# borglab/gtsfm

Hardware: NVIDIA H100
Metric: image_pairs_per_sec (higher is better)
Workload: dtype f32

## Files before the change

gtsfm_b200/_lib.py:

```python
from __future__ import annotations

import ctypes as C
from pathlib import Path
from typing import Optional

import numpy as np

LIB_PATH = Path(__file__).resolve().parent / "libgtsfm_b200.so"

_lib: Optional[C.CDLL] = None


class B200Error(RuntimeError):
    pass


class LightGlueParams(C.Structure):
    _fields_ = [("depth_confidence", C.c_double), ("width_confidence", C.c_double), ("filter_threshold", C.c_double),
                ("prune_min_kpts", C.c_int), ("fp16_attention", C.c_int)]


class LightGluePair(C.Structure):
    _fields_ = [("kp0", C.c_void_p), ("desc0", C.c_void_p), ("n0", C.c_int), ("kp1", C.c_void_p), ("desc1", C.c_void_p), ("n1", C.c_int),
                ("out_matches", C.c_void_p), ("out_scores", C.c_void_p), ("out_k", C.c_int), ("out_stop_layer", C.c_int),
# ... 128 lines not shown
class TwoViewEvalResult(C.Structure):
    _fields_ = [("num_rows", C.c_int), ("num_inliers_gt", C.c_int), ("no_gt", C.c_int), ("no_rows", C.c_int),
                ("inlier_avg_reproj_error_gt", C.c_double), ("outlier_avg_reproj_error_gt", C.c_double),
                ("R_error_deg", C.c_double), ("U_error_deg", C.c_double)]


class ViewGraphParams(C.Structure):
    _fields_ = [("criterion", C.c_int), ("pad_", C.c_int), ("error_threshold_deg", C.c_double)]


VG_MEDIAN, VG_MIN = 0, 1

_vp, _i, _f, _sz = C.c_void_p, C.c_int, C.c_float, C.c_size_t
_ip = C.POINTER(C.c_int)

SIGNATURES = {
    "b2_version": (_i, []),
    "b2_create": (_i, [_i, C.POINTER(_vp)]),
    "b2_destroy": (None, [_vp]),
    "b2_last_error": (C.c_char_p, [_vp]),
    "b2_launch_count": (C.c_uint64, [_vp]),
    "b2_h2d_bytes": (C.c_uint64, [_vp]),
    "b2_set_option": (C.c_int, [_vp, C.c_char_p, C.c_int64]),
    "b2_profile_start": (_i, [_vp, C.c_char_p]),
    "b2_profile_stop": (_i, [_vp, C.POINTER(C.c_double), C.POINTER(C.c_uint64), C.POINTER(C.c_double)]),
    "b2_debug_fetch": (C.c_int64, [_vp, C.c_char_p, _vp, C.c_int64]),
    "b2_debug_linear_host": (_i, [_vp, C.POINTER(LinearLaunch), C.POINTER(LinearProblem), _i]),
    "b2_debug_conv_host": (_i, [_vp, C.POINTER(ConvLayer)]),
    "b2_debug_gemm_segments_host": (_i, [_vp, _vp, _vp, _vp, _i, _i, _i, _i, _vp, _vp, _i, _vp, _vp]),
    "b2_debug_attention_host": (_i, [_vp, _i, _ip, _ip, _i, _f, _i, _vp, _vp, _vp, _vp]),
    "b2_debug_superglue_assign_host": (_i, [_vp, _i, _i, _vp, _i, _i, _f, _i, _f, _vp, _vp, _vp, _vp, _vp, _vp, _vp, _ip, _ip]),
    "b2_debug_lightglue_assign_host": (_i, [_vp, _i, _i, _vp, _i, _i, _vp, _vp, _vp, _vp, _f, _vp, _vp, _vp, _vp, _vp, _vp, _vp, _ip,
                                            _ip]),
    "b2_debug_lightglue_argmax_host": (_i, [_vp, _i, _vp, _i, _i, _vp, _vp, _vp, _vp, _vp, _ip]),
    "b2_debug_lightglue_posenc_host": (_i, [_vp, _i, _vp, _vp, _vp, _vp, _vp, _vp]),
    "b2_debug_lightglue_ln_gelu_host": (_i, [_vp, _i, _vp, _vp, _vp, _vp, _vp, _vp]),
    "b2_debug_lightglue_rowheads_host": (_i, [_vp, _i, _vp, _vp, _vp, _vp, _vp, _vp, _vp, _vp, _vp, _vp]),
    "b2_debug_lightglue_prune_host": (_i, [_vp, _i, _vp, _vp, _vp, _f, _f, _vp, _vp]),
    "b2_debug_lightglue_gather_host": (_i, [_vp, _i, _vp, _vp, _vp, _vp, _vp, _vp, _vp, _vp, _vp, _vp, _vp, _vp, _vp]),
    "b2_debug_lightglue_filter_host": (_i, [_vp, _i, _i, _vp, _vp, _vp, _f, _vp, _vp, _vp, _vp, _ip]),
    "b2_superpoint_set_weights": (_i, [_vp, _vp, _sz]),
    "b2_superpoint_detect_dev": (_i, [_vp, _vp, _i, _i, _i, _sz, _f, _i, _i, _vp, _vp, _i, _ip, C.POINTER(C.c_uint64), _vp]),
    "b2_superpoint_describe_dev": (_i, [_vp, C.c_uint64, _vp, _i, _vp, _vp]),
    "b2_superpoint_extract_dev": (_i, [_vp, _vp, _i, _i, _i, _sz, _f, _i, _i, _i, _vp, _vp, _vp, _ip, _vp]),
    "b2_superpoint_extract_async_dev": (_i, [_vp, _vp, _i, _i, _i, _sz, _f, _i, _i, _i, _vp, _vp, _vp, _vp, _vp]),
    "b2_superpoint_finish_dev": (_i, [_vp, _vp]),
    "b2_superpoint_detect_host": (_i, [_vp, _vp, _i, _i, _i, _f, _i, _i, _vp, _vp, _i, _ip, C.POINTER(C.c_uint64)]),
    "b2_superpoint_describe_host": (_i, [_vp, C.c_uint64, _vp, _i, _vp]),
    "b2_image_resize_dev": (_i, [_vp, _vp, _i, _i, _i, _sz, _vp, _i, _i, _vp]),
    "b2_lightglue_set_weights": (_i, [_vp, _vp, _sz]),
    "b2_lightglue_qkv_rows": (_i, [_vp]),
    "b2_lightglue_match_dev": (_i, [_vp, _vp, _vp, _i, _vp, _vp, _i, C.POINTER(LightGlueParams), _vp, _vp, _ip, _ip, _vp]),
    "b2_lightglue_match_host": (_i, [_vp, _vp, _vp, _i, _vp, _vp, _i, C.POINTER(LightGlueParams), _vp, _vp, _ip, _ip]),
    "b2_lightglue_match_batched_dev": (_i, [_vp, C.POINTER(LightGluePair), _i, C.POINTER(LightGlueParams), _vp]),
    "b2_lightglue_trace_count": (_i, [_vp]),
    "b2_lightglue_trace_get": (_i, [_vp, _i, _vp, _vp, _vp, _vp, _vp, _vp]),
    "b2_lightglue_encoded_bytes": (_sz, [_i]),
    "b2_lightglue_encode_batched_dev": (_i, [_vp, C.POINTER(LightGlueImage), _i, C.POINTER(LightGlueParams), _vp]),
    "b2_superglue_set_weights": (_i, [_vp, _vp, _sz]),
    "b2_superglue_match_dev": (_i, [_vp, _vp, _vp, _vp, _i, _i, _i, _vp, _vp, _vp, _i, _i, _i, _i, _f, _vp, _vp, _ip, _vp]),
    "b2_superglue_match_host": (_i, [_vp, _vp, _vp, _vp, _i, _i, _i, _vp, _vp, _vp, _i, _i, _i, _i, _f, _vp, _vp, _ip]),
    "b2_superglue_trace_count": (_i, [_vp]),
    "b2_superglue_trace_get": (_i, [_vp, _i, _vp, _vp]),
    "b2_netvlad_blob_floats": (_sz, []),
    "b2_netvlad_set_weights": (_i, [_vp, _vp, _sz]),
    "b2_netvlad_describe_dev": (_i, [_vp, _vp, _i, _i, _i, _vp, _vp]),
# ... 136 lines not shown
```

gtsfm_b200/csrc/lightglue.cu:

```cuda
#include <stdlib.h>

#include "common.cuh"
#include "linear.cuh"
#include "assign_ps.cuh"

namespace {
constexpr int LG_LAYERS = 9;
constexpr size_t LG_NFLOATS = 11851601;
constexpr int D = 256;

struct SelfW {
  float *wqkv, *bqkv, *wout, *bout, *w0, *b0, *lng, *lnb, *w3, *b3;
};
struct CrossW {
  float *wqv, *bqv, *wout, *bout, *w0, *b0, *lng, *lnb, *w3, *b3;
};
struct AssignW {
  float *wm, *bm, *wf, *bf;
};
struct ConfW {
  float *w, *b;
};
}

// ... 7 lines not shown
  int n = 0;
  int cap = 0;
};

struct LgPair {
  bool active = false;
  int n0 = 0, n1 = 0;
  int stop = 0;
  long long* out_matches = nullptr;
  float* out_scores = nullptr;
};

struct LgTraceRec {
  int pair = 0, side = 0, layer = 0, n = 0;
  int heads = 0;
  int unconf = 0, kept = 0, stop = 0;
  std::vector<float> x, conf, mat;
  std::vector<int> ind, keep;
};

struct LightGlueState {
  bool loaded = false;
  int persist_ctas = 132;
  DevBuf wblob, wblob_h, wblob_l, errflag;
  bool use_tc = true;
  float* wr = nullptr;
  SelfW sw[LG_LAYERS];
  CrossW cw[LG_LAYERS];
  AssignW aw[LG_LAYERS];
  ConfW tw[LG_LAYERS - 1];
  float thr[LG_LAYERS];
  LgSide side[LG_MAX_SIDES];
  LgPair pair[LG_MAX_PAIRS];
  DevBuf sim[LG_MAX_PAIRS], counters, attn_part, attn_ml, attn_cnt, as_part, as_bar;
  HostBuf hread;
  std::vector<LgTraceRec> trace;
};

template <typename J>
struct JobList {
  J j[LG_MAX_SIDES];
};

void lg_destroy(b2_context* ctx) {
  delete ctx->lg;
  ctx->lg = nullptr;
}


struct PosJob {
  const float* kp;
  int n;
  float *cs, *sn;
  int* ind;
};
__global__ void __launch_bounds__(1024) k_lg_posenc(const __grid_constant__ JobList<PosJob> jobs, const float* __restrict__ wr ) {
  const PosJob& jb = jobs.j[blockIdx.y];
  const float* __restrict__ kp = jb.kp;
  const int n = jb.n;
  float* __restrict__ cs = jb.cs;
  float* __restrict__ sn = jb.sn;
  int* __restrict__ ind = jb.ind;
  if (n <= 0 || blockIdx.x * 1024 >= n * 32) return;
  __shared__ float red[4][32];
  __shared__ float bb[4];
  float mnx = INFINITY, mny = INFINITY, mxx = -INFINITY, mxy = -INFINITY;
  for (int i = threadIdx.x; i < n; i += blockDim.x) {
// ... 365 lines not shown
  if (j < n) {
    const float cm = cmax[j], cl = clog[j], l1 = l1g[j];
    for (int i0 = warp; i0 < m; i0 += LG_COL_WARPS * LG_COL_UNROLL) {
      float x[LG_COL_UNROLL], rm[LG_COL_UNROLL], rl[LG_COL_UNROLL], l0[LG_COL_UNROLL];
#pragma unroll
      for (int u = 0; u < LG_COL_UNROLL; ++u) {
        const int i = i0 + u * LG_COL_WARPS;
        const bool in = i < m;
        x[u] = in ? sim[(size_t)i * n + j] : 0.f;
        rm[u] = in ? rmax[i] : 0.f, rl[u] = in ? rlog[i] : 0.f, l0[u] = in ? l0g[i] : 0.f;
      }
#pragma unroll
      for (int u = 0; u < LG_COL_UNROLL; ++u) {
        const int i = i0 + u * LG_COL_WARPS;
        if (i < m) {
          const float sc = (((x[u] - rm[u]) - rl[u]) + ((x[u] - cm) - cl)) + (l0[u] + l1);
          if (sc > bv) bv = sc, bi = i;
        }
      }
    }
  }
  sv[warp][lane] = bv, si[warp][lane] = bi;
  __syncthreads();
  if (warp == 0 && j < n) {
    for (int w = 1; w < LG_COL_WARPS; ++w) {
      float ov = sv[w][lane];
      int oi = si[w][lane];
      if (ov > bv || (ov == bv && oi < bi)) bv = ov, bi = oi;
    }
    arg[j] = bi == 0x7fffffff ? 0 : bi;
  }
}

__global__ void __launch_bounds__(1024) k_lg_filter(const float* __restrict__ best0, const int* __restrict__ a0,
                                                     const int* __restrict__ a1, int m, float th, const int* __restrict__ ind0,
                                                     const int* __restrict__ ind1, long long* __restrict__ out,
                                                     float* __restrict__ outs, int* __restrict__ count) {
  __shared__ int wtot[32];
  __shared__ int carry;
  if (threadIdx.x == 0) carry = 0;
  __syncthreads();
  const int lane = threadIdx.x & 31, warp = threadIdx.x >> 5;
  for (int base = 0; base < m; base += 1024) {
    int i = base + threadIdx.x;
    bool valid = false;
    float ms = 0.f;
    int j = 0;
    if (i < m) {
      j = a0[i];
      bool mutual = a1[j] == i;
      ms = mutual ? expf(best0[i]) : 0.f;
      valid = mutual && best0[i] > -INFINITY && ms > th;
    }
    unsigned vm = __ballot_sync(0xffffffffu, valid);
    if (lane == 0) wtot[warp] = __popc(vm);
    __syncthreads();
    if (warp == 0) {
      int w = wtot[lane], ws = w;
#pragma unroll
      for (int o = 1; o < 32; o <<= 1) {
        int u = __shfl_up_sync(0xffffffffu, ws, o);
        if (lane >= o) ws += u;
      }
      wtot[lane] = ws - w;
    }
    __syncthreads();
    int pos = carry + wtot[warp] + __popc(vm & ((1u << lane) - 1));
    if (valid) {
      out[2 * (size_t)pos] = ind0[i];
      out[2 * (size_t)pos + 1] = ind1[j];
      if (outs) outs[pos] = ms;
    }
    __syncthreads();
    if (threadIdx.x == 1023) carry = pos + (valid ? 1 : 0);
    __syncthreads();
  }
  if (threadIdx.x == 0) *count = carry;
}


struct LgStats {
  float *max, *log, *lsg;
};
struct LgAssign {
  const float* sim;
  int M, N;
  const float *z0, *z1;
  const int *ind0, *ind1;
  float thr;
  LgStats r, c;
  float* best0;
  int *arg0, *arg1;
  DevBuf *part, *bar;
  int* err_flag;
  long long* out_matches;
  float* out_scores;
  int* count;
};

static int lg_assign_argmax(b2_context* ctx, cudaStream_t st, const LgAssign& p, int path, int G, int* ran) {
  const float* sim = p.sim;
  const int M = p.M, N = p.N;
  const bool persistent = path == 0 ? assign_ps_fits(1, N) : path == 1;
  if (persistent && !assign_ps_fits(1, N)) return b2_fail(ctx, B2_ERR_ARG, "the persistent assignment kernel holds at most 6240 columns");
  if (ran) *ran = persistent ? 1 : 2;
  int rc;
  if (persistent) {
    B2_CUDA(ctx, p.part->ensure((size_t)G * 2 * N * sizeof(float)));
    B2_CUDA(ctx, p.bar->ensure(16));
    B2_CUDA(ctx, cudaMemsetAsync(p.bar->p, 0, 16, st));
    SinkArgs sa{};
    sa.Z = sim, sa.M = M, sa.N = N, sa.iters = 1, sa.u = p.r.max, sa.v = p.c.max;
    sa.rlog = p.r.log, sa.clog = p.c.log, sa.z0 = p.z0, sa.z1 = p.z1;
    sa.lsg0 = p.r.lsg, sa.lsg1 = p.c.lsg, sa.part = p.part->as<float>(), sa.bar = p.bar->as<unsigned>();
    sa.best0 = p.best0, sa.arg0 = p.arg0, sa.arg1 = p.arg1, sa.err_flag = p.err_flag;
    if ((rc = launch_assign_ps<1>(ctx, st, sa, G, "k_lg_assign"))) return rc;
  } else {
    B2_LAUNCH(ctx, k_lg_row_stats, cdiv(M, 8), 256, 0, st, sim, M, N, p.r.max, p.r.log, p.z0, p.r.lsg);
    B2_CHECK_LAUNCH(ctx);
    B2_LAUNCH(ctx, k_lg_col_stats, cdiv(N, 32), 1024, 0, st, sim, M, N, p.c.max, p.c.log, p.z1, p.c.lsg);
    B2_CHECK_LAUNCH(ctx);
    B2_LAUNCH(ctx, k_lg_row_argmax, cdiv(M, 8), 256, 0, st, sim, M, N, p.r.max, p.r.log, p.c.max, p.c.log, p.r.lsg, p.c.lsg, p.best0,
              p.arg0);
    B2_CHECK_LAUNCH(ctx);
    B2_LAUNCH(ctx, k_lg_col_argmax, cdiv(N, 32), 1024, 0, st, sim, M, N, p.r.max, p.r.log, p.c.max, p.c.log, p.r.lsg, p.c.lsg, p.arg1);
    B2_CHECK_LAUNCH(ctx);
  }
  return B2_OK;
}

static int lg_assign(b2_context* ctx, cudaStream_t st, const LgAssign& p, int path, int G, int* ran) {
  const int M = p.M;
  int rc;
  if ((rc = lg_assign_argmax(ctx, st, p, path, G, ran))) return rc;
  B2_LAUNCH(ctx, k_lg_filter, 1, 1024, 0, st, p.best0, p.arg0, p.arg1, M, p.thr, p.ind0, p.ind1, p.out_matches, p.out_scores, p.count);
  B2_CHECK_LAUNCH(ctx);
  return B2_OK;
}

extern "C" int b2_lightglue_qkv_rows(int* out) {
  if (!out) return B2_ERR_ARG;
  for (int r = 0; r < 3 * D; ++r) out[r] = (r % D) * 3 + r / D;
  return B2_OK;
}

extern "C" int b2_lightglue_set_weights(b2_context* ctx, const float* blob, size_t n_floats) {
  if (!ctx || !blob) return B2_ERR_ARG;
  std::lock_guard<std::mutex> lk(ctx->mu);
  if (n_floats != LG_NFLOATS)
    return b2_fail(ctx, B2_ERR_ARG, "lightglue blob must hold 11851601 floats, got " + std::to_string(n_floats));
  cudaSetDevice(ctx->device);
  if (!ctx->lg) ctx->lg = new LightGlueState();
  LightGlueState* s = ctx->lg;
  std::vector<size_t> sizes;
  sizes.push_back(64);
  for (int i = 0; i < LG_LAYERS; ++i) {
    const size_t self_sz[] = {768 * 256, 768, 256 * 256, 256, 512 * 512, 512, 512, 512, 256 * 512, 256};
    const size_t cross_sz[] = {256 * 256, 256, 256 * 256, 256, 256 * 256, 256, 512 * 512, 512, 512, 512, 256 * 512, 256};
    for (size_t z : self_sz) sizes.push_back(z);
    for (size_t z : cross_sz) sizes.push_back(z);
  }
  for (int i = 0; i < LG_LAYERS; ++i) {
    const size_t asz[] = {256, 1, 256 * 256, 256};
    for (size_t z : asz) sizes.push_back(z);
  }
  for (int i = 0; i < LG_LAYERS - 1; ++i) sizes.push_back(256), sizes.push_back(1);
  constexpr int SELF_T = 10, LAYER_T = 22;
  std::vector<size_t> order(sizes.size());
// ... 399 lines not shown
    int ns = 0, mx = 0;
    for (int li = 0; li < nlive; ++li) {
      if (s->pair[live[li]].stop != layer) continue;
      for (int side = 0; side < 2; ++side) {
        LgSide& sd = s->side[2 * live[li] + side];
        const float* x = sd.x[sd.cur].as<float>();
        LinArgs& a = g[ns];
        a.a1f = x, a.a1p = planes_of(sd.xs[sd.cur], (size_t)sd.cap * 256), a.lda1 = 256, a.K1 = 256, a.w = s->aw[layer].wf, a.ldb = 256;
        a.bias = s->aw[layer].bf, a.scale = 0.25f;
        a.cf = sd.md.as<float>(), a.ldc = 256, a.cp = planes_of(sd.md, (size_t)sd.cap * 256), a.ldch = 256, a.M = sd.n, a.N = 256;
        hj.j[ns] = {x, sd.n, s->aw[layer].wm, s->aw[layer].bm, nullptr, nullptr, sd.ls.as<float>()};
        mx = sd.n > mx ? sd.n : mx;
        ++ns;
      }
    }
    if (ns == 0) continue;
    if ((rc = run_linear(ctx, st, tw, g, ns, "lg_assign_proj"))) return rc;
    B2_LAUNCH(ctx, k_lg_rowheads, dim3(cdiv(mx, 8), ns), 256, 0, st, hj, (const float*)nullptr, (const float*)nullptr);
    B2_CHECK_LAUNCH(ctx);
  }
  {
    LinArgs gs[LG_MAX_PAIRS];
    for (int li = 0; li < nlive; ++li) {
      const int p = live[li];
      LgSide &a = s->side[2 * p], &b = s->side[2 * p + 1];
      B2_CUDA(ctx, s->sim[p].ensure((size_t)a.n * b.n * 4));
      LinArgs& g = gs[li];
      g.a1f = a.md.as<float>(), g.a1p = planes_of(a.md, (size_t)a.cap * 256), g.lda1 = 256, g.K1 = 256;
      g.bf = b.md.as<float>(), g.bp = planes_of(b.md, (size_t)b.cap * 256), g.ldb = 256;
      g.cf = s->sim[p].as<float>(), g.ldc = b.n, g.tc_want_f32 = true, g.M = a.n, g.N = b.n;
    }
    if ((rc = run_linear(ctx, st, tw, gs, nlive, "lg_assign_sim"))) return rc;
  }
  for (int li = 0; li < nlive; ++li) {
    const int p = live[li];
    LgSide &a = s->side[2 * p], &b = s->side[2 * p + 1];
    const LgAssign la{s->sim[p].as<float>(), a.n, b.n, a.ls.as<float>(), b.ls.as<float>(), a.ind[a.cur].as<int>(), b.ind[b.cur].as<int>(),
                      (float)prm->filter_threshold, {a.rmax.as<float>(), a.rlog.as<float>(), a.lsg.as<float>()},
                      {b.rmax.as<float>(), b.rlog.as<float>(), b.lsg.as<float>()}, a.amax.as<float>(), a.aidx.as<int>(), b.aidx.as<int>(),
                      &s->as_part, &s->as_bar, s->errflag.as<int>(), s->pair[p].out_matches, s->pair[p].out_scores,
                      counters + 4 * LG_MAX_PAIRS + p};
    if ((rc = lg_assign(ctx, st, la, 0, s->persist_ctas, nullptr))) return rc;
  }
  B2_CUDA(ctx, cudaMemcpyAsync(hread + 4 * LG_MAX_PAIRS, counters + 4 * LG_MAX_PAIRS, LG_MAX_PAIRS * sizeof(int), cudaMemcpyDeviceToHost, st));
  B2_CUDA(ctx, cudaMemcpyAsync(hread + 5 * LG_MAX_PAIRS, s->errflag.p, sizeof(int), cudaMemcpyDeviceToHost, st));
  B2_CUDA(ctx, cudaStreamSynchronize(st));
  if (s->use_tc && hread[5 * LG_MAX_PAIRS]) return b2_fail(ctx, B2_ERR_STATE, "wgmma pipeline timed out on an mbarrier (kernel bug)");
  for (int li = 0; li < nlive; ++li) pairs[live[li]].out_k = hread[4 * LG_MAX_PAIRS + live[li]];
  ctx->debug["lg_desc0"] = {s->side[0].x[s->side[0].cur].as<float>(), (int64_t)s->side[0].n * 256};
  ctx->debug["lg_desc1"] = {s->side[1].x[s->side[1].cur].as<float>(), (int64_t)s->side[1].n * 256};
  return B2_OK;
}

static int lg_match_pairs(b2_context* ctx, b2_lightglue_pair* pairs, int n_pairs, const b2_lightglue_params* prm, cudaStream_t st) {
  LightGlueState* s = ctx->lg;
  if (!s || !s->loaded) return b2_fail(ctx, B2_ERR_STATE, "lightglue weights not set");
  s->persist_ctas = ctx->sm_count - ctx->reserve_sms > 0 ? ctx->sm_count - ctx->reserve_sms : 1;
  s->trace.clear();
  const int bmax = ctx->lg_batch > 0 && ctx->lg_batch < LG_MAX_PAIRS ? ctx->lg_batch : LG_MAX_PAIRS;
  for (int p0 = 0; p0 < n_pairs; p0 += bmax) {
    const int np = n_pairs - p0 < bmax ? n_pairs - p0 : bmax;
    int rc = lg_match_batch(ctx, pairs + p0, np, prm, st, p0);
    if (rc) return rc;
  }
  return B2_OK;
}

extern "C" int b2_lightglue_match_batched_dev(b2_context* ctx, b2_lightglue_pair* pairs, int n_pairs, const b2_lightglue_params* params,
                                              void* stream) {
  if (!ctx || !params || n_pairs < 0 || (n_pairs > 0 && !pairs)) return B2_ERR_ARG;
  for (int p = 0; p < n_pairs; ++p) {
    const b2_lightglue_pair& pr = pairs[p];
    if (pr.n0 < 0 || pr.n1 < 0) return B2_ERR_ARG;
    if (pr.n0 > 0 && pr.n1 > 0 && (!pr.kp0 || !pr.desc0 || !pr.kp1 || !pr.desc1 || !pr.out_matches)) return B2_ERR_ARG;
    if (((uintptr_t)pr.enc0 | (uintptr_t)pr.enc1) & 15) return B2_ERR_ARG;
  }
// ... 175 lines not shown
  std::vector<int> iota((size_t)(M > N ? M : N));
  for (size_t i = 0; i < iota.size(); ++i) iota[i] = (int)i;
  B2_CUDA(ctx, cudaMemcpyAsync(dsim.p, sim, (size_t)M * N * 4, cudaMemcpyHostToDevice, st));
  B2_CUDA(ctx, cudaMemcpyAsync(dz0.p, z0, (size_t)M * 4, cudaMemcpyHostToDevice, st));
  B2_CUDA(ctx, cudaMemcpyAsync(dz1.p, z1, (size_t)N * 4, cudaMemcpyHostToDevice, st));
  B2_CUDA(ctx, cudaMemcpyAsync(di0.p, ind0 ? ind0 : iota.data(), (size_t)M * 4, cudaMemcpyHostToDevice, st));
  B2_CUDA(ctx, cudaMemcpyAsync(di1.p, ind1 ? ind1 : iota.data(), (size_t)N * 4, cudaMemcpyHostToDevice, st));
  B2_CUDA(ctx, cudaMemsetAsync(err.p, 0, 16, st));
  const int G = ctas > 0 ? ctas : (ctx->sm_count - ctx->reserve_sms > 0 ? ctx->sm_count - ctx->reserve_sms : 1);
  float *r = rs.as<float>(), *c = cs.as<float>();
  const LgAssign p{dsim.as<float>(), M, N, dz0.as<float>(), dz1.as<float>(), di0.as<int>(), di1.as<int>(), threshold, {r, r + M, r + 2 * M},
                   {c, c + N, c + 2 * N}, dbest.as<float>(), da0.as<int>(), da1.as<int>(), &part, &bar, err.as<int>(),
                   out.as<long long>(), outs.as<float>(), cnt.as<int>()};
  const int rc = lg_assign(ctx, st, p, path, G, out_path);
  if (rc) return rc;
  int k = 0, e = 0;
  B2_CUDA(ctx, cudaMemcpyAsync(&k, cnt.p, 4, cudaMemcpyDeviceToHost, st));
  B2_CUDA(ctx, cudaMemcpyAsync(&e, err.p, 4, cudaMemcpyDeviceToHost, st));
  B2_CUDA(ctx, cudaMemcpyAsync(row_stats, rs.p, (size_t)3 * M * 4, cudaMemcpyDeviceToHost, st));
  B2_CUDA(ctx, cudaMemcpyAsync(col_stats, cs.p, (size_t)3 * N * 4, cudaMemcpyDeviceToHost, st));
  B2_CUDA(ctx, cudaMemcpyAsync(best0, dbest.p, (size_t)M * 4, cudaMemcpyDeviceToHost, st));
  B2_CUDA(ctx, cudaMemcpyAsync(arg0, da0.p, (size_t)M * 4, cudaMemcpyDeviceToHost, st));
  B2_CUDA(ctx, cudaMemcpyAsync(arg1, da1.p, (size_t)N * 4, cudaMemcpyDeviceToHost, st));
  B2_CUDA(ctx, cudaStreamSynchronize(st));
  if (k > 0) {
    B2_CUDA(ctx, cudaMemcpy(out_matches, out.p, (size_t)k * 16, cudaMemcpyDeviceToHost));
    B2_CUDA(ctx, cudaMemcpy(out_scores, outs.p, (size_t)k * 4, cudaMemcpyDeviceToHost));
  }
  *out_k = k;
  if (e) return b2_fail(ctx, B2_ERR_STATE, "the persistent assignment kernel timed out in its grid barrier (kernel bug)");
  return B2_OK;
}


extern "C" int b2_lightglue_trace_count(b2_context* ctx) {
  if (!ctx) return B2_ERR_ARG;
  std::lock_guard<std::mutex> lk(ctx->mu);
  return ctx->lg ? (int)ctx->lg->trace.size() : 0;
}

extern "C" int b2_lightglue_trace_get(b2_context* ctx, int i, int* meta, float* x, int* ind, float* conf, float* mat, int* keep) {
  if (!ctx || !meta) return B2_ERR_ARG;
  std::lock_guard<std::mutex> lk(ctx->mu);
  if (!ctx->lg || i < 0 || i >= (int)ctx->lg->trace.size()) return b2_fail(ctx, B2_ERR_ARG, "no such lightglue trace record");
  const LgTraceRec& r = ctx->lg->trace[i];
  const int m[8] = {r.pair, r.side, r.layer, r.n, r.heads, r.unconf, r.kept, r.stop};
  memcpy(meta, m, sizeof(m));
  if (x) memcpy(x, r.x.data(), r.x.size() * 4);
  if (ind) memcpy(ind, r.ind.data(), r.ind.size() * 4);
  if (conf) memcpy(conf, r.conf.data(), r.conf.size() * 4);
  if (mat) memcpy(mat, r.mat.data(), r.mat.size() * 4);
  if (keep) memcpy(keep, r.keep.data(), r.keep.size() * 4);
  return B2_OK;
}


constexpr size_t LG_DBG_GUARD = 4096;

struct LgDbg {
  b2_context* ctx;
  cudaStream_t st;
  std::vector<std::unique_ptr<DevBuf>> bufs;
  struct Out {
    void* host;
    size_t bytes;
    const DevBuf* d;
// ... 162 lines not shown
        (rc = d.put(cs + 32 * (size_t)o, 32 * m, false, &dcs)) || (rc = d.put(sn + 32 * (size_t)o, 32 * m, false, &dsn)) ||
        (rc = d.put(ind + o, m, false, &di)) || (rc = d.put(x2 + 256 * (size_t)o, 256 * m, true, &j.x2)) ||
        (rc = d.put(cs2 + 32 * (size_t)o, 32 * m, true, &j.cs2)) || (rc = d.put(sn2 + 32 * (size_t)o, 32 * m, true, &j.sn2)) ||
        (rc = d.put(ind2 + o, m, true, &j.ind2)) ||
        (planes && ((rc = d.put(planes + 512 * (size_t)o, 512 * m, false, &dp)) || (rc = d.put(planes2 + 512 * (size_t)o, 512 * m, true, &dp2)))))
      return rc;
    j.src = ds, j.cnt = dcnt + i, j.n = n[i], j.x = dx, j.cs = dcs, j.sn = dsn, j.ind = di;
    j.ph = reinterpret_cast<const __half*>(dp), j.pstride = 256 * m, j.ph2 = reinterpret_cast<__half*>(dp2), j.pstride2 = 256 * m;
  }
  if (mx > 0) {
    B2_LAUNCH(ctx, k_lg_gather, dim3(cdiv(mx, 8), np), 256, 0, d.st, gj);
    B2_CHECK_LAUNCH(ctx);
  }
  return d.finish("b2_debug_lightglue_gather_host");
}

extern "C" int b2_debug_lightglue_filter_host(b2_context* ctx, int m, int n, const float* best0, const int* a0, const int* a1, float th,
                                              const int* ind0, const int* ind1, int64_t* out_matches, float* out_scores, int* out_k) {
  if (!ctx || m <= 0 || n <= 0 || !best0 || !a0 || !a1 || !ind0 || !ind1 || !out_matches || !out_scores || !out_k) return B2_ERR_ARG;
  for (int i = 0; i < m; ++i)
    if (a0[i] < 0 || a0[i] >= n) return b2_fail(ctx, B2_ERR_ARG, "b2_debug_lightglue_filter_host: a0 entry out of range");
  std::lock_guard<std::mutex> lk(ctx->mu);
  cudaSetDevice(ctx->device);
  LgDbg d{ctx, ctx->stream};
  float *db, *dos;
  int *da0, *da1, *di0, *di1, *dk;
  int64_t* dom;
  int rc;
  if ((rc = d.put(best0, (size_t)m, false, &db)) || (rc = d.put(a0, (size_t)m, false, &da0)) || (rc = d.put(a1, (size_t)n, false, &da1)) ||
      (rc = d.put(ind0, (size_t)m, false, &di0)) || (rc = d.put(ind1, (size_t)n, false, &di1)) ||
      (rc = d.put(out_matches, 2 * (size_t)m, true, &dom)) || (rc = d.put(out_scores, (size_t)m, true, &dos)) ||
      (rc = d.put(out_k, 1, true, &dk)))
    return rc;
  B2_LAUNCH(ctx, k_lg_filter, 1, 1024, 0, d.st, db, da0, da1, m, th, di0, di1, reinterpret_cast<long long*>(dom), dos, dk);
  B2_CHECK_LAUNCH(ctx);
  return d.finish("b2_debug_lightglue_filter_host");
}

extern "C" int b2_debug_lightglue_argmax_host(b2_context* ctx, int path, const float* sim, int M, int N, const float* z0, const float* z1,
                                              float* best0, int* arg0, int* arg1, int* out_path) {
  if (!ctx || !sim || !z0 || !z1 || !best0 || !arg0 || !arg1 || !out_path || M <= 0 || N <= 0 || path < 0 || path > 2) return B2_ERR_ARG;
  std::lock_guard<std::mutex> lk(ctx->mu);
  cudaSetDevice(ctx->device);
  LgDbg d{ctx, ctx->stream};
  DevBuf stats, part, bar, err;
  float *dsim, *dz0, *dz1, *db;
  int *da0, *da1;
  int rc;
  if ((rc = d.put(sim, (size_t)M * N, false, &dsim)) || (rc = d.put(z0, (size_t)M, false, &dz0)) || (rc = d.put(z1, (size_t)N, false, &dz1)) ||
      (rc = d.put(best0, (size_t)M, true, &db)) || (rc = d.put(arg0, (size_t)M, true, &da0)) || (rc = d.put(arg1, (size_t)N, true, &da1)))
    return rc;
  B2_CUDA(ctx, stats.ensure((size_t)3 * (M + N) * 4));
  B2_CUDA(ctx, err.ensure(16));
  B2_CUDA(ctx, cudaMemsetAsync(err.p, 0, 16, d.st));
  float *r = stats.as<float>(), *c = r + 3 * M;
  const LgAssign p{dsim, M, N, dz0, dz1, nullptr, nullptr, 0.f, {r, r + M, r + 2 * M}, {c, c + N, c + 2 * N}, db, da0, da1, &part, &bar,
                   err.as<int>(), nullptr, nullptr, nullptr};
  const int G = ctx->sm_count - ctx->reserve_sms > 0 ? ctx->sm_count - ctx->reserve_sms : 1;
  if ((rc = lg_assign_argmax(ctx, d.st, p, path, G, out_path))) return rc;
  if ((rc = d.finish("b2_debug_lightglue_argmax_host"))) return rc;
  int e = 0;
  B2_CUDA(ctx, cudaMemcpy(&e, err.p, 4, cudaMemcpyDeviceToHost));
  if (e) return b2_fail(ctx, B2_ERR_STATE, "the persistent assignment kernel timed out in its grid barrier (kernel bug)");
  return B2_OK;
}
```

include/gtsfm_b200.h:

```cpp
#ifndef GTSFM_B200_H
#define GTSFM_B200_H

#include <stddef.h>
#include <stdint.h>

#ifdef __cplusplus
extern "C" {
#endif

typedef struct b2_context b2_context;

int b2_version(void);
int b2_create(int device, b2_context** out);
void b2_destroy(b2_context* ctx);
const char* b2_last_error(const b2_context* ctx);
uint64_t b2_launch_count(const b2_context* ctx);
uint64_t b2_h2d_bytes(const b2_context* ctx);
int b2_set_option(b2_context* ctx, const char* name, int64_t value);
int b2_profile_start(b2_context* ctx, const char* kernel_prefix);
int b2_profile_stop(b2_context* ctx, double* total_ms, uint64_t* launches, double* work);
int64_t b2_debug_fetch(b2_context* ctx, const char* name, float* host_out, int64_t max_floats);

typedef struct b2_linear_problem {
  const float* a1; int lda1;
// ... 6 lines not shown
} b2_linear_problem;
typedef struct b2_linear_launch {
  int path;
  int k1, k2, per_problem_b;
  const float* bias;
  float scale;
  int relu, gelu, head_major, lo_unscaled;
  int resid_in_place;
} b2_linear_launch;
int b2_debug_linear_host(b2_context* ctx, const b2_linear_launch* launch, const b2_linear_problem* problems, int np);
typedef struct b2_conv_layer {
  int path;
  int dilation, pool, relu, ctas;
  int height, width, cin, cout;
  const float* in;
  const float* weight;
  const float* bias;
  float* out;
  uint16_t* out_hi; uint16_t* out_lo;
} b2_conv_layer;
int b2_debug_conv_host(b2_context* ctx, const b2_conv_layer* layer);
int b2_debug_gemm_segments_host(b2_context* ctx, const float* A, const float* B, const float* bias, int M, int K, int nseg,
                                int rot_mask, const float* cs, const float* sn, int separate, uint16_t* out_hi,
                                uint16_t* out_lo);
int b2_debug_attention_host(b2_context* ctx, int np, const int* nq, const int* nk, int heads, float scale, int single,
                            const float* q, const float* k, const float* v, float* o);
int b2_debug_superglue_assign_host(b2_context* ctx, int path, int ctas, const float* Z, int M, int N, float alpha, int iters,
                                   float threshold, float* u, float* v, float* best0, int* arg0, int* arg1, uint32_t* out_matches,
                                   float* out_scores, int* out_k, int* out_path);
int b2_debug_lightglue_assign_host(b2_context* ctx, int path, int ctas, const float* sim, int M, int N, const float* z0,
                                   const float* z1, const int* ind0, const int* ind1, float threshold, float* row_stats,
                                   float* col_stats, float* best0, int* arg0, int* arg1, int64_t* out_matches, float* out_scores,
                                   int* out_k, int* out_path);
int b2_debug_lightglue_argmax_host(b2_context* ctx, int path, const float* sim, int M, int N, const float* z0, const float* z1,
                                   float* best0, int* arg0, int* arg1, int* out_path);
int b2_debug_lightglue_posenc_host(b2_context* ctx, int np, const int* n, const float* kp, const float* wr, float* cs, float* sn,
                                   int* ind);
int b2_debug_lightglue_ln_gelu_host(b2_context* ctx, int np, const int* n, const float* g, const float* b, float* h, uint16_t* hi,
                                    uint16_t* lo);
int b2_debug_lightglue_rowheads_host(b2_context* ctx, int np, const int* n, const int* mode, const float* x, const float* w1,
                                     const float* b1, const float* w2, const float* b2, float* o1, float* o2, float* zraw);
int b2_debug_lightglue_prune_host(b2_context* ctx, int np, const int* n, const float* conf, const float* mat, float thr,
                                  float keep_thr, int* src, int* counters);
int b2_debug_lightglue_gather_host(b2_context* ctx, int np, const int* n, const int* cnt, const int* src, const float* x,
                                   const float* cs, const float* sn, const int* ind, const uint16_t* planes, float* x2, float* cs2,
                                   float* sn2, int* ind2, uint16_t* planes2);
int b2_debug_lightglue_filter_host(b2_context* ctx, int m, int n, const float* best0, const int* a0, const int* a1, float th,
                                   const int* ind0, const int* ind1, int64_t* out_matches, float* out_scores, int* out_k);

int b2_superpoint_set_weights(b2_context* ctx, const float* host_blob, size_t n_floats);

int b2_superpoint_detect_dev(b2_context* ctx, const uint8_t* image, int height, int width, int channels, size_t pitch,
                             float keypoint_threshold, int nms_radius, int border, float* out_xy, float* out_score,
                             int cap, int* out_n, uint64_t* out_map_token, void* stream);
int b2_superpoint_describe_dev(b2_context* ctx, uint64_t map_token, const float* xy, int n, float* out_desc, void* stream);
int b2_superpoint_extract_dev(b2_context* ctx, const uint8_t* image, int height, int width, int channels, size_t pitch,
                              float keypoint_threshold, int nms_radius, int border, int max_keypoints, float* out_xy,
                              float* out_score, float* out_desc, int* out_n, void* stream);
int b2_superpoint_extract_async_dev(b2_context* ctx, const uint8_t* image, int height, int width, int channels, size_t pitch,
                                    float threshold, int nms_radius, int border, int max_keypoints, float* out_xy,
                                    float* out_score, float* out_desc, int* out_n_pinned, void* stream);
int b2_superpoint_finish_dev(b2_context* ctx, void* stream);

int b2_superpoint_detect_host(b2_context* ctx, const uint8_t* image, int height, int width, int channels,
                              float keypoint_threshold, int nms_radius, int border, float* out_xy, float* out_score,
                              int cap, int* out_n, uint64_t* out_map_token);
// ... 352 lines not shown
```

Before: 131.2.

## Batch LightGlue assignment across pairs with strip-tiled sweep and merge kernels

Replaces the per-pair assignment loop (a persistent argmax path plus one filter launch per pair) with one batched pipeline for all live pairs. Column-strip by row-tile tasks stream the similarity matrix through cp.async smem rings and compute online log-sum-exp partials, a merge kernel reduces them, a second sweep computes argmax partials, and a batched filter kernel runs all pairs in one launch. The aim is to cut launch count and grid-sync overhead and to fill the GPU with several pairs at once. The cost is extra partial-buffer traffic and a second full read of the similarity matrix.

```diff
diff --git a/gtsfm_b200/_lib.py b/gtsfm_b200/_lib.py
--- a/gtsfm_b200/_lib.py
+++ b/gtsfm_b200/_lib.py
@@ -184,6 +184,8 @@
     "b2_debug_superglue_assign_host": (_i, [_vp, _i, _i, _vp, _i, _i, _f, _i, _f, _vp, _vp, _vp, _vp, _vp, _vp, _vp, _ip, _ip]),
     "b2_debug_lightglue_assign_host": (_i, [_vp, _i, _i, _vp, _i, _i, _vp, _vp, _vp, _vp, _f, _vp, _vp, _vp, _vp, _vp, _vp, _vp, _ip,
                                             _ip]),
+    "b2_debug_lightglue_assign_batched_host": (_i, [_vp, _i, _vp, _vp, _vp, _vp, _vp, _vp, _vp, _f, _vp, _vp, _vp, _vp, _vp, _vp, _vp,
+                                                    _vp]),
     "b2_debug_lightglue_argmax_host": (_i, [_vp, _i, _vp, _i, _i, _vp, _vp, _vp, _vp, _vp, _ip]),
     "b2_debug_lightglue_posenc_host": (_i, [_vp, _i, _vp, _vp, _vp, _vp, _vp, _vp]),
     "b2_debug_lightglue_ln_gelu_host": (_i, [_vp, _i, _vp, _vp, _vp, _vp, _vp, _vp]),
diff --git a/gtsfm_b200/csrc/lightglue.cu b/gtsfm_b200/csrc/lightglue.cu
--- a/gtsfm_b200/csrc/lightglue.cu
+++ b/gtsfm_b200/csrc/lightglue.cu
@@ -63,7 +63,7 @@
   float thr[LG_LAYERS];
   LgSide side[LG_MAX_SIDES];
   LgPair pair[LG_MAX_PAIRS];
-  DevBuf sim[LG_MAX_PAIRS], counters, attn_part, attn_ml, attn_cnt, as_part, as_bar;
+  DevBuf sim[LG_MAX_PAIRS], counters, attn_part, attn_ml, attn_cnt, as_part;
   HostBuf hread;
   std::vector<LgTraceRec> trace;
 };
@@ -495,10 +495,27 @@
   }
 }
 
-__global__ void __launch_bounds__(1024) k_lg_filter(const float* __restrict__ best0, const int* __restrict__ a0,
-                                                     const int* __restrict__ a1, int m, float th, const int* __restrict__ ind0,
-                                                     const int* __restrict__ ind1, long long* __restrict__ out,
-                                                     float* __restrict__ outs, int* __restrict__ count) {
+struct FilterJob {
+  const float* best0;
+  const int *a0, *a1;
+  int m;
+  float th;
+  const int *ind0, *ind1;
+  long long* out;
+  float* outs;
+  int* count;
+};
+__global__ void __launch_bounds__(1024) k_lg_filter(const __grid_constant__ JobList<FilterJob> jobs) {
+  const FilterJob& jb = jobs.j[blockIdx.y];
+  const float* __restrict__ best0 = jb.best0;
+  const int* __restrict__ a0 = jb.a0;
+  const int* __restrict__ a1 = jb.a1;
+  const int* __restrict__ ind0 = jb.ind0;
+  const int* __restrict__ ind1 = jb.ind1;
+  long long* __restrict__ out = jb.out;
+  float* __restrict__ outs = jb.outs;
+  const int m = jb.m;
+  const float th = jb.th;
   __shared__ int wtot[32];
   __shared__ int carry;
   if (threadIdx.x == 0) carry = 0;
@@ -538,7 +555,176 @@
     if (threadIdx.x == 1023) carry = pos + (valid ? 1 : 0);
     __syncthreads();
   }
-  if (threadIdx.x == 0) *count = carry;
+  if (threadIdx.x == 0) *jb.count = carry;
+}
+
+constexpr int AS_T = 256, AS_WARPS = AS_T / 32;
+constexpr int AS_KW = 4;
+constexpr int AS_STRIP = 32 * 4 * AS_KW;
+constexpr int AS_H = 32;
+constexpr int AS_ROWS = AS_WARPS * AS_H;
+constexpr int AS_S = 4;
+constexpr int AS_NONE = 0x7fffffff;
+constexpr size_t AS_DSMEM = (size_t)(AS_WARPS * AS_S + 3) * AS_STRIP * sizeof(float);
+static_assert(AS_S >= 2 && AS_H == 32, "the column partials fit in the rings; a warp holds one row's constants per lane");
+
+struct AsgJob {
+  const float* sim;
+  int M, N;
+  const float *z0, *z1;
+  float *rmax, *rlog, *lsg0, *cmax, *clog, *lsg1;
+  float* best0;
+  int *arg0, *arg1;
+  float2 *rpart, *cpart;
+  int task0, strips;
+};
+struct AsgBatch {
+  AsgJob j[LG_MAX_PAIRS];
+  int n, tasks;
+};
+
+template <int MODE>
+__global__ void __launch_bounds__(AS_T, 3) k_lg_asg_sweep(const __grid_constant__ AsgBatch b) {
+  extern __shared__ __align__(16) float as_smem[];
+  const int lane = threadIdx.x & 31, warp = threadIdx.x >> 5;
+  float* ring = as_smem + (size_t)warp * AS_S * AS_STRIP;
+  float2(*cpw)[AS_STRIP] = reinterpret_cast<float2(*)[AS_STRIP]>(as_smem);
+  float(*cc)[AS_STRIP] = reinterpret_cast<float(*)[AS_STRIP]>(as_smem + (size_t)AS_WARPS * AS_S * AS_STRIP);
+  for (int t0 = blockIdx.x; t0 < b.tasks; t0 += gridDim.x) {
+    const int task = MODE == 0 ? t0 : b.tasks - 1 - t0;
+    int p = 0;
+    while (p + 1 < b.n && task >= b.j[p + 1].task0) ++p;
+    const AsgJob& jb = b.j[p];
+    const int M = jb.M, N = jb.N;
+    const int local = task - jb.task0, strip = local % jb.strips, tile = local / jb.strips;
+    const int c0 = strip * AS_STRIP, cn = min(AS_STRIP, N - c0);
+    const int rb = tile * AS_ROWS + warp * AS_H, re = min(M, rb + AS_H);
+    if (MODE == 1) {
+      for (int q = threadIdx.x; q < cn; q += AS_T) cc[0][q] = jb.cmax[c0 + q], cc[1][q] = jb.clog[c0 + q], cc[2][q] = jb.lsg1[c0 + q];
+      __syncthreads();
+    }
+    const bool vec = (N & 3) == 0;
+    const float* src = jb.sim + c0;
+    auto issue = [&](int r, int slot) {
+      if (r < re) {
+        const float* row = src + (size_t)r * N;
+        float* dst = ring + slot * AS_STRIP;
+#pragma unroll
+        for (int k = 0; k < AS_KW; ++k) {
+          const int q = 4 * (lane + 32 * k);
+          if (vec) {
+            if (q < cn)
+              asm volatile("cp.async.cg.shared.global [%0], [%1], 16;" ::"r"((uint32_t)__cvta_generic_to_shared(dst + q)), "l"(row + q) : "memory");
+          } else {
+#pragma unroll
+            for (int c = 0; c < 4; ++c)
+              if (q + c < cn)
+                asm volatile("cp.async.ca.shared.global [%0], [%1], 4;" ::"r"((uint32_t)__cvta_generic_to_shared(dst + q + c)), "l"(row + q + c)
+                             : "memory");
+          }
+        }
+      }
+      asm volatile("cp.async.commit_group;" ::: "memory");
+    };
+    float rcv[3] = {0.f, 0.f, 0.f};
+    if (MODE == 1 && rb + lane < re) rcv[0] = jb.rmax[rb + lane], rcv[1] = jb.rlog[rb + lane], rcv[2] = jb.lsg0[rb + lane];
+    float ca[4 * AS_KW], cb[4 * AS_KW];
+#pragma unroll
+    for (int e = 0; e < 4 * AS_KW; ++e) ca[e] = -INFINITY, cb[e] = MODE == 0 ? 0.f : __int_as_float(AS_NONE);
+    if (rb < re) {
+      for (int s = 0; s < AS_S - 1; ++s) issue(rb + s, s);
+      for (int r = rb; r < re; ++r) {
+        issue(r + AS_S - 1, (r - rb + AS_S - 1) % AS_S);
+        asm volatile("cp.async.wait_group %0;" ::"n"(AS_S - 1) : "memory");
+        __syncwarp();
+        const float* buf = ring + ((r - rb) % AS_S) * AS_STRIP;
+        float x[4 * AS_KW];
+#pragma unroll
+        for (int k = 0; k < AS_KW; ++k) {
+          const int q = 4 * (lane + 32 * k);
+          const float4 v = q < cn ? *reinterpret_cast<const float4*>(buf + q) : make_float4(0.f, 0.f, 0.f, 0.f);
+          x[4 * k] = v.x, x[4 * k + 1] = v.y, x[4 * k + 2] = v.z, x[4 * k + 3] = v.w;
+        }
+        __syncwarp();
+        float rm = 0.f, rl = 0.f, l0 = 0.f;
+        if (MODE == 1) {
+          rm = __shfl_sync(0xffffffffu, rcv[0], r - rb), rl = __shfl_sync(0xffffffffu, rcv[1], r - rb);
+          l0 = __shfl_sync(0xffffffffu, rcv[2], r - rb);
+        }
+        float m = -INFINITY, s = 0.f;
+        int bi = AS_NONE;
+#pragma unroll
+        for (int e = 0; e < 4 * AS_KW; ++e) {
+          const int q = 4 * (lane + 32 * (e >> 2)) + (e & 3);
+          if (q >= cn) continue;
+          const float z = x[e];
+          if (MODE == 0) {
+            sk_online(m, s, z);
+            sk_online(ca[e], cb[e], z);
+          } else {
+            const float sc = (((z - rm) - rl) + ((z - cc[0][q]) - cc[1][q])) + (l0 + cc[2][q]);
+            if (sc > m) m = sc, bi = c0 + q;
+            if (sc > ca[e]) ca[e] = sc, cb[e] = __int_as_float(r);
+          }
+        }
+#pragma unroll
+        for (int o = 16; o > 0; o >>= 1) {
+          const float m2 = __shfl_xor_sync(0xffffffffu, m, o);
+          if (MODE == 0) {
+            const float s2 = __shfl_xor_sync(0xffffffffu, s, o);
+            sk_merge(m, s, m2, s2);
+          } else {
+            const int i2 = __shfl_xor_sync(0xffffffffu, bi, o);
+            if (m2 > m || (m2 == m && i2 < bi)) m = m2, bi = i2;
+          }
+        }
+        if (lane == 0) jb.rpart[(size_t)strip * M + r] = make_float2(m, MODE == 0 ? s : __int_as_float(bi));
+      }
+      asm volatile("cp.async.wait_group 0;" ::: "memory");
+    }
+    __syncthreads();
+#pragma unroll
+    for (int e = 0; e < 4 * AS_KW; ++e) {
+      const int q = 4 * (lane + 32 * (e >> 2)) + (e & 3);
+      if (q < cn) cpw[warp][q] = make_float2(ca[e], cb[e]);
+    }
+    __syncthreads();
+    for (int q = threadIdx.x; q < cn; q += AS_T) {
+      float2 acc = cpw[0][q];
+      for (int w = 1; w < AS_WARPS; ++w) {
+        const float2 o = cpw[w][q];
+        if (MODE == 0) sk_merge(acc.x, acc.y, o.x, o.y);
+        else if (o.x > acc.x) acc = o;
+      }
+      jb.cpart[(size_t)tile * N + c0 + q] = acc;
+    }
+    __syncthreads();
+  }
+}
+
+template <int MODE>
+__global__ void __launch_bounds__(256) k_lg_asg_merge(const __grid_constant__ AsgBatch b) {
+  const AsgJob& jb = b.j[blockIdx.y];
+  const int M = jb.M, N = jb.N;
+  const int t = blockIdx.x * 256 + threadIdx.x;
+  if (t >= M + N) return;
+  const bool row = t < M;
+  const int idx = row ? t : t - M, parts = row ? jb.strips : (M + AS_ROWS - 1) / AS_ROWS, stride = row ? M : N;
+  const float2* part = (row ? jb.rpart : jb.cpart) + idx;
+  float m = -INFINITY, s = MODE == 0 ? 0.f : __int_as_float(AS_NONE);
+  for (int g = 0; g < parts; ++g) {
+    const float2 o = part[(size_t)g * stride];
+    if (MODE == 0) sk_merge(m, s, o.x, o.y);
+    else if (o.x > m) m = o.x, s = o.y;
+  }
+  if (MODE == 0) {
+    if (row) jb.rmax[idx] = m, jb.rlog[idx] = logf(s), jb.lsg0[idx] = sk_logsigmoid(jb.z0[idx]);
+    else jb.cmax[idx] = m, jb.clog[idx] = logf(s), jb.lsg1[idx] = sk_logsigmoid(jb.z1[idx]);
+  } else {
+    const int bi = __float_as_int(s) == AS_NONE ? 0 : __float_as_int(s);
+    if (row) jb.best0[idx] = m, jb.arg0[idx] = bi;
+    else jb.arg1[idx] = bi;
+  }
 }
 
 
@@ -592,11 +778,66 @@
   return B2_OK;
 }
 
+static FilterJob lg_filter_job(const LgAssign& p) {
+  return {p.best0, p.arg0, p.arg1, p.M > 0 && p.N > 0 ? p.M : 0, p.thr, p.ind0, p.ind1, p.out_matches, p.out_scores, p.count};
+}
+
 static int lg_assign(b2_context* ctx, cudaStream_t st, const LgAssign& p, int path, int G, int* ran) {
-  const int M = p.M;
   int rc;
   if ((rc = lg_assign_argmax(ctx, st, p, path, G, ran))) return rc;
-  B2_LAUNCH(ctx, k_lg_filter, 1, 1024, 0, st, p.best0, p.arg0, p.arg1, M, p.thr, p.ind0, p.ind1, p.out_matches, p.out_scores, p.count);
+  JobList<FilterJob> fj{};
+  fj.j[0] = lg_filter_job(p);
+  B2_LAUNCH(ctx, k_lg_filter, 1, 1024, 0, st, fj);
+  B2_CHECK_LAUNCH(ctx);
+  return B2_OK;
+}
+
+static int lg_assign_batch(b2_context* ctx, cudaStream_t st, const LgAssign* p, int n, int G, DevBuf& part) {
+  AsgBatch b{};
+  JobList<FilterJob> fj{};
+  size_t np2 = 0;
+  int mx = 0;
+  double bytes = 0.0;
+  for (int k = 0; k < n; ++k) {
+    const int M = p[k].M > 0 && p[k].N > 0 ? p[k].M : 0, N = M > 0 ? p[k].N : 0;
+    np2 += (size_t)cdiv(N, AS_STRIP) * M + (size_t)cdiv(M, AS_ROWS) * N;
+    mx = M + N > mx ? M + N : mx;
+    bytes += (double)M * N * 4.0;
+  }
+  B2_CUDA(ctx, part.ensure((np2 > 0 ? np2 : 1) * sizeof(float2)));
+  float2* pp = part.as<float2>();
+  for (int k = 0; k < n; ++k) {
+    const LgAssign& a = p[k];
+    AsgJob& j = b.j[k];
+    const int M = a.M > 0 && a.N > 0 ? a.M : 0, N = M > 0 ? a.N : 0;
+    j = {a.sim, M, N, a.z0, a.z1, a.r.max, a.r.log, a.r.lsg, a.c.max, a.c.log, a.c.lsg, a.best0, a.arg0, a.arg1, pp, nullptr, b.tasks, cdiv(N, AS_STRIP)};
+    pp += (size_t)j.strips * M;
+    j.cpart = pp;
+    pp += (size_t)cdiv(M, AS_ROWS) * N;
+    b.tasks += j.strips * cdiv(M, AS_ROWS);
+    fj.j[k] = lg_filter_job(a);
+  }
+  b.n = n;
+  if (b.tasks > 0) {
+    int fit[2];
+    B2_CUDA(ctx, cudaFuncSetAttribute(k_lg_asg_sweep<0>, cudaFuncAttributeMaxDynamicSharedMemorySize, (int)AS_DSMEM));
+    B2_CUDA(ctx, cudaFuncSetAttribute(k_lg_asg_sweep<1>, cudaFuncAttributeMaxDynamicSharedMemorySize, (int)AS_DSMEM));
+    B2_CUDA(ctx, cudaOccupancyMaxActiveBlocksPerMultiprocessor(&fit[0], k_lg_asg_sweep<0>, AS_T, AS_DSMEM));
+    B2_CUDA(ctx, cudaOccupancyMaxActiveBlocksPerMultiprocessor(&fit[1], k_lg_asg_sweep<1>, AS_T, AS_DSMEM));
+    const int per_sm = fit[0] < fit[1] ? fit[0] : fit[1];
+    if (per_sm < 1) return b2_fail(ctx, B2_ERR_STATE, "k_lg_asg_sweep does not fit on an SM");
+    const int grid = b.tasks < per_sm * G ? b.tasks : per_sm * G;
+    b2_prof_work(ctx, "k_lg_asg_sweep", 2.0 * bytes);
+    B2_LAUNCH(ctx, k_lg_asg_sweep<0>, grid, AS_T, AS_DSMEM, st, b);
+    B2_CHECK_LAUNCH(ctx);
+    B2_LAUNCH(ctx, k_lg_asg_merge<0>, dim3(cdiv(mx, 256), n), 256, 0, st, b);
+    B2_CHECK_LAUNCH(ctx);
+    B2_LAUNCH(ctx, k_lg_asg_sweep<1>, grid, AS_T, AS_DSMEM, st, b);
+    B2_CHECK_LAUNCH(ctx);
+    B2_LAUNCH(ctx, k_lg_asg_merge<1>, dim3(cdiv(mx, 256), n), 256, 0, st, b);
+    B2_CHECK_LAUNCH(ctx);
+  }
+  B2_LAUNCH(ctx, k_lg_filter, dim3(1, n), 1024, 0, st, fj);
   B2_CHECK_LAUNCH(ctx);
   return B2_OK;
 }
@@ -1062,16 +1303,16 @@
     }
     if ((rc = run_linear(ctx, st, tw, gs, nlive, "lg_assign_sim"))) return rc;
   }
+  LgAssign la[LG_MAX_PAIRS];
   for (int li = 0; li < nlive; ++li) {
     const int p = live[li];
     LgSide &a = s->side[2 * p], &b = s->side[2 * p + 1];
-    const LgAssign la{s->sim[p].as<float>(), a.n, b.n, a.ls.as<float>(), b.ls.as<float>(), a.ind[a.cur].as<int>(), b.ind[b.cur].as<int>(),
-                      (float)prm->filter_threshold, {a.rmax.as<float>(), a.rlog.as<float>(), a.lsg.as<float>()},
-                      {b.rmax.as<float>(), b.rlog.as<float>(), b.lsg.as<float>()}, a.amax.as<float>(), a.aidx.as<int>(), b.aidx.as<int>(),
-                      &s->as_part, &s->as_bar, s->errflag.as<int>(), s->pair[p].out_matches, s->pair[p].out_scores,
-                      counters + 4 * LG_MAX_PAIRS + p};
-    if ((rc = lg_assign(ctx, st, la, 0, s->persist_ctas, nullptr))) return rc;
-  }
+    la[li] = {s->sim[p].as<float>(), a.n, b.n, a.ls.as<float>(), b.ls.as<float>(), a.ind[a.cur].as<int>(), b.ind[b.cur].as<int>(),
+              (float)prm->filter_threshold, {a.rmax.as<float>(), a.rlog.as<float>(), a.lsg.as<float>()},
+              {b.rmax.as<float>(), b.rlog.as<float>(), b.lsg.as<float>()}, a.amax.as<float>(), a.aidx.as<int>(), b.aidx.as<int>(),
+              nullptr, nullptr, nullptr, s->pair[p].out_matches, s->pair[p].out_scores, counters + 4 * LG_MAX_PAIRS + p};
+  }
+  if ((rc = lg_assign_batch(ctx, st, la, nlive, s->persist_ctas, s->as_part))) return rc;
   B2_CUDA(ctx, cudaMemcpyAsync(hread + 4 * LG_MAX_PAIRS, counters + 4 * LG_MAX_PAIRS, LG_MAX_PAIRS * sizeof(int), cudaMemcpyDeviceToHost, st));
   B2_CUDA(ctx, cudaMemcpyAsync(hread + 5 * LG_MAX_PAIRS, s->errflag.p, sizeof(int), cudaMemcpyDeviceToHost, st));
   B2_CUDA(ctx, cudaStreamSynchronize(st));
@@ -1313,6 +1554,77 @@
   return B2_OK;
 }
 
+extern "C" int b2_debug_lightglue_assign_batched_host(b2_context* ctx, int n, const int* M, const int* N, const float* sim,
+                                                      const float* z0, const float* z1, const int* ind0, const int* ind1,
+                                                      float threshold, float* row_stats, float* col_stats, float* best0, int* arg0,
+                                                      int* arg1, int64_t* out_matches, float* out_scores, int* out_k) {
+  if (!ctx || !M || !N || !sim || !z0 || !z1 || !row_stats || !col_stats || !best0 || !arg0 || !arg1 || !out_matches || !out_scores ||
+      !out_k || n < 1 || n > LG_MAX_PAIRS)
+    return B2_ERR_ARG;
+  size_t sm = 0, sn = 0, ssim = 0;
+  size_t om[LG_MAX_PAIRS], on[LG_MAX_PAIRS], osim[LG_MAX_PAIRS];
+  for (int k = 0; k < n; ++k) {
+    if (M[k] < 0 || N[k] < 0) return B2_ERR_ARG;
+    om[k] = sm, on[k] = sn, osim[k] = ssim;
+    sm += M[k], sn += N[k], ssim += (size_t)M[k] * N[k];
+  }
+  std::lock_guard<std::mutex> lk(ctx->mu);
+  cudaSetDevice(ctx->device);
+  cudaStream_t st = ctx->stream;
+  DevBuf dsim[LG_MAX_PAIRS], dz0, dz1, di0, di1, rs, cs, dbest, da0, da1, out, outs, cnt, part;
+  auto up = [&](DevBuf& d, const void* h, size_t bytes) -> cudaError_t {
+    cudaError_t e = d.ensure(bytes > 16 ? bytes : 16);
+    if (e == cudaSuccess && bytes) e = h ? cudaMemcpyAsync(d.p, h, bytes, cudaMemcpyHostToDevice, st) : cudaMemsetAsync(d.p, 0xff, bytes, st);
+    return e;
+  };
+  std::vector<int> iota0(sm), iota1(sn);
+  for (int k = 0; k < n; ++k) {
+    for (int i = 0; i < M[k]; ++i) iota0[om[k] + i] = i;
+    for (int j = 0; j < N[k]; ++j) iota1[on[k] + j] = j;
+  }
+  for (int k = 0; k < n; ++k) B2_CUDA(ctx, up(dsim[k], sim + osim[k], (size_t)M[k] * N[k] * 4));
+  B2_CUDA(ctx, up(dz0, z0, sm * 4));
+  B2_CUDA(ctx, up(dz1, z1, sn * 4));
+  B2_CUDA(ctx, up(di0, ind0 ? ind0 : iota0.data(), sm * 4));
+  B2_CUDA(ctx, up(di1, ind1 ? ind1 : iota1.data(), sn * 4));
+  B2_CUDA(ctx, up(rs, nullptr, 3 * sm * 4));
+  B2_CUDA(ctx, up(cs, nullptr, 3 * sn * 4));
+  B2_CUDA(ctx, up(dbest, nullptr, sm * 4));
+  B2_CUDA(ctx, up(da0, nullptr, sm * 4));
+  B2_CUDA(ctx, up(da1, nullptr, sn * 4));
+  B2_CUDA(ctx, up(out, nullptr, sm * 16));
+  B2_CUDA(ctx, up(outs, nullptr, sm * 4));
+  B2_CUDA(ctx, up(cnt, nullptr, (size_t)n * 4));
+  LgAssign p[LG_MAX_PAIRS];
+  float *r = rs.as<float>(), *c = cs.as<float>();
+  for (int k = 0; k < n; ++k) {
+    float *rk = r + 3 * om[k], *ck = c + 3 * on[k];
+    p[k] = {dsim[k].as<float>(), M[k], N[k], dz0.as<float>() + om[k], dz1.as<float>() + on[k], di0.as<int>() + om[k], di1.as<int>() + on[k],
+            threshold, {rk, rk + M[k], rk + 2 * M[k]}, {ck, ck + N[k], ck + 2 * N[k]}, dbest.as<float>() + om[k], da0.as<int>() + om[k],
+            da1.as<int>() + on[k], nullptr, nullptr, nullptr, out.as<long long>() + 2 * om[k], outs.as<float>() + om[k], cnt.as<int>() + k};
+  }
+  const int G = ctx->sm_count - ctx->reserve_sms > 0 ? ctx->sm_count - ctx->reserve_sms : 1;
+  int rc;
+  if ((rc = lg_assign_batch(ctx, st, p, n, G, part))) return rc;
+  std::vector<int> k(n);
+  B2_CUDA(ctx, cudaMemcpyAsync(k.data(), cnt.p, (size_t)n * 4, cudaMemcpyDeviceToHost, st));
+  B2_CUDA(ctx, cudaMemcpyAsync(row_stats, rs.p, 3 * sm * 4, cudaMemcpyDeviceToHost, st));
+  B2_CUDA(ctx, cudaMemcpyAsync(col_stats, cs.p, 3 * sn * 4, cudaMemcpyDeviceToHost, st));
+  B2_CUDA(ctx, cudaMemcpyAsync(best0, dbest.p, sm * 4, cudaMemcpyDeviceToHost, st));
+  B2_CUDA(ctx, cudaMemcpyAsync(arg0, da0.p, sm * 4, cudaMemcpyDeviceToHost, st));
+  B2_CUDA(ctx, cudaMemcpyAsync(arg1, da1.p, sn * 4, cudaMemcpyDeviceToHost, st));
+  B2_CUDA(ctx, cudaStreamSynchronize(st));
+  for (int q = 0; q < n; ++q) {
+    if (k[q] < 0 || k[q] > M[q]) return b2_fail(ctx, B2_ERR_STATE, "b2_debug_lightglue_assign_batched_host: match count out of range");
+    out_k[q] = k[q];
+    if (k[q] > 0) {
+      B2_CUDA(ctx, cudaMemcpy(out_matches + 2 * om[q], out.as<long long>() + 2 * om[q], (size_t)k[q] * 16, cudaMemcpyDeviceToHost));
+      B2_CUDA(ctx, cudaMemcpy(out_scores + om[q], outs.as<float>() + om[q], (size_t)k[q] * 4, cudaMemcpyDeviceToHost));
+    }
+  }
+  return B2_OK;
+}
+
 
 extern "C" int b2_lightglue_trace_count(b2_context* ctx) {
   if (!ctx) return B2_ERR_ARG;
@@ -1541,7 +1853,9 @@
       (rc = d.put(out_matches, 2 * (size_t)m, true, &dom)) || (rc = d.put(out_scores, (size_t)m, true, &dos)) ||
       (rc = d.put(out_k, 1, true, &dk)))
     return rc;
-  B2_LAUNCH(ctx, k_lg_filter, 1, 1024, 0, d.st, db, da0, da1, m, th, di0, di1, reinterpret_cast<long long*>(dom), dos, dk);
+  JobList<FilterJob> fj{};
+  fj.j[0] = {db, da0, da1, m, th, di0, di1, reinterpret_cast<long long*>(dom), dos, dk};
+  B2_LAUNCH(ctx, k_lg_filter, 1, 1024, 0, d.st, fj);
   B2_CHECK_LAUNCH(ctx);
   return d.finish("b2_debug_lightglue_filter_host");
 }
diff --git a/include/gtsfm_b200.h b/include/gtsfm_b200.h
--- a/include/gtsfm_b200.h
+++ b/include/gtsfm_b200.h
@@ -62,6 +62,10 @@
                                    const float* z1, const int* ind0, const int* ind1, float threshold, float* row_stats,
                                    float* col_stats, float* best0, int* arg0, int* arg1, int64_t* out_matches, float* out_scores,
                                    int* out_k, int* out_path);
+int b2_debug_lightglue_assign_batched_host(b2_context* ctx, int n, const int* M, const int* N, const float* sim, const float* z0,
+                                           const float* z1, const int* ind0, const int* ind1, float threshold, float* row_stats,
+                                           float* col_stats, float* best0, int* arg0, int* arg1, int64_t* out_matches,
+                                           float* out_scores, int* out_k);
 int b2_debug_lightglue_argmax_host(b2_context* ctx, int path, const float* sim, int M, int N, const float* z0, const float* z1,
                                    float* best0, int* arg0, int* arg1, int* out_path);
 int b2_debug_lightglue_posenc_host(b2_context* ctx, int np, const int* n, const float* kp, const float* wr, float* cs, float* sn,
```

Measured after the change: 134.2, median of 6. 1.02x the previous value.
